# anilkeshwani/speech-integration

Measured on AMD Instinct MI355X. Metric: train_tokens_per_sec, higher is better.
Workload: dtype bf16; 1 GPU; Llama-3.2-1B +5000 DSUs (V=133258), SFT step fwd+bwd+AdamW, seq_len=2048, batch=8/GPU, grad_accum=1, 16 layers, random-init weights, MLS-shaped synthetic DSU sequences; global_batch=8, seq_len=2048, parallelism=dp1

## Files before the change

include/ssi_hip.h:

```cpp
#ifndef SSI_HIP_H
#define SSI_HIP_H

#include <stdint.h>

#ifdef __cplusplus
extern "C" {
#endif

#define SSI_ABI_VERSION 9

enum { SSI_F32 = 0, SSI_BF16 = 1 };
enum { SSI_OK = 0, SSI_ERR_ARG = 1, SSI_ERR_UNSUPPORTED = 2, SSI_ERR_WORKSPACE = 3, SSI_ERR_HIP = 1000  };
enum { SSI_GEMM_NT = 0, SSI_GEMM_NN = 1, SSI_GEMM_TN = 2 };
enum { SSI_TILES_STATIC = 0, SSI_TILES_DYNAMIC = 1 };
int ssi_set_gemm_tile_order(int mode);

enum { SSI_IMPL_AUTO = 0, SSI_IMPL_GENERIC = 1, SSI_IMPL_MFMA = 2,
       SSI_IMPL_MFMA_WG8 = 3  };

int ssi_abi_version(void);
const char* ssi_last_error(void);
int ssi_set_impl(int impl);

int ssi_embed_fwd(const int64_t* tokens, const void* table, void* out, int64_t n_tok, int64_t dim, int64_t vocab,
                  int dtype, void* stream);
int64_t ssi_embed_bwd_workspace_bytes(int64_t vocab);
int ssi_embed_bwd(const int64_t* tokens, const void* dout, void* dtable, int64_t n_tok, int64_t dim, int64_t vocab,
                  int dtype, void* workspace, int64_t workspace_bytes, void* stream);

int ssi_rmsnorm_fwd(const void* x, const void* scale, void* y, float* rstd, int64_t rows, int64_t dim, float eps,
                    int dtype, void* stream);
int64_t ssi_rmsnorm_bwd_workspace_bytes(int64_t rows, int64_t dim);
int ssi_rmsnorm_bwd(const void* dy, const void* x, const void* scale, const float* rstd, const void* dres, void* dx,
                    void* dscale, int accumulate_dscale, int64_t rows, int64_t dim, int dtype, void* workspace,
                    int64_t workspace_bytes, void* stream);

int ssi_rope_inplace(void* x, int64_t ld, int64_t rows, int64_t seq_len, int n_heads_rot, int head_dim,
                     const float* table, int64_t table_len, const int32_t* positions, int inverse, int dtype,
                     void* stream);

int ssi_gemm_rope(int64_t M, int64_t N, int64_t K, const void* A, int64_t lda, const void* B, int64_t ldb, void* C, int64_t ldc,
                  int64_t seq_len, int n_heads_rot, int head_dim, const float* rope_table, int64_t table_len,
                  const int32_t* positions, int dtype, void* stream);

int ssi_attn_fwd(const void* qkv, int64_t ld, void* out, float* lse, int64_t batch, int64_t seq, int n_heads,
                 int n_kv, int head_dim, int dtype, void* stream);
int ssi_attn_bwd(const void* qkv, int64_t ld, const void* out, const void* dout, const float* lse, void* dqkv,
                 float* delta, int64_t batch, int64_t seq, int n_heads, int n_kv, int head_dim, int dtype,
                 void* stream);

int ssi_attn_varlen_fwd(const void* qkv, int64_t ld, void* out, float* lse, const int32_t* doc_start, const int32_t* doc_end,
                        int64_t batch, int64_t seq, int n_heads, int n_kv, int head_dim, int dtype, void* stream);
int ssi_attn_varlen_bwd(const void* qkv, int64_t ld, const void* out, const void* dout, const float* lse, void* dqkv,
                        float* delta, const int32_t* doc_start, const int32_t* doc_end, int64_t batch, int64_t seq,
                        int n_heads, int n_kv, int head_dim, int dtype, void* stream);

int ssi_doc_ranges(const int64_t* input_pos, int64_t batch, int64_t seq, int64_t max_pos, int32_t* positions, int32_t* doc_start,
                   int32_t* doc_end, int32_t* n_clamped, void* stream);

// ... 81 lines not shown
```

speech-integration_amd/csrc/embed_ce.hip:

```cpp
#include "common_hip.h"

template <typename T>
__global__ __launch_bounds__(256) void embed_fwd_kernel(const int64_t* __restrict__ tokens, const T* __restrict__ table,
                                                        T* __restrict__ out, int64_t n_tok, int dim, int64_t vocab) {
    constexpr int N = Vec16<T>::N;
    const int nvec = dim / N;
    for (int64_t t = blockIdx.x; t < n_tok; t += gridDim.x) {
        const int64_t tok = tokens[t];
        const bool ok = tok >= 0 && tok < vocab;
        for (int v = threadIdx.x; v < nvec; v += 256) {
            Vec16<T> a;
            if (ok) a = load16(table + tok * dim + v * N);
            else
#pragma unroll
                for (int i = 0; i < N; ++i) a.set(i, 0.f);
            store16(out + t * dim + v * N, a);
        }
    }
}

extern "C" int ssi_embed_fwd(const int64_t* tokens, const void* table, void* out, int64_t n_tok, int64_t dim,
                             int64_t vocab, int dtype, void* stream) {
    if (n_tok == 0) return SSI_OK;
    SSI_CHECK_ARG(tokens && table && out && n_tok > 0 && dim > 0 && dim % 8 == 0 && vocab > 0);
    const unsigned grid = (unsigned)(n_tok < 65536 ? n_tok : 65536);
    SSI_DISPATCH_DTYPE(dtype, hipLaunchKernelGGL(embed_fwd_kernel<T>, dim3(grid), dim3(256), 0, (hipStream_t)stream, tokens,
                                                 (const T*)table, (T*)out, n_tok, (int)dim, vocab));
    SSI_LAUNCH_CHECK();
    return SSI_OK;
}

__global__ __launch_bounds__(256) void embed_index_kernel(const int64_t* __restrict__ tokens, int64_t n_tok, int64_t vocab,
                                                          int* __restrict__ first, int* __restrict__ count) {
    const int64_t t = (int64_t)blockIdx.x * 256 + threadIdx.x;
    if (t >= n_tok) return;
    const int64_t tok = tokens[t];
    if (tok < 0 || tok >= vocab) return;
    atomicMin(&first[tok], (int)t);
    atomicAdd(&count[tok], 1);
}

template <typename T, int MAXV>
__global__ __launch_bounds__(256) void embed_bwd_kernel(const int64_t* __restrict__ tokens, const T* __restrict__ dout,
                                                        T* __restrict__ dtable, int64_t n_tok, int dim, int64_t vocab,
                                                        const int* __restrict__ first, const int* __restrict__ count) {
    constexpr int N = Vec16<T>::N;
    const int lane = threadIdx.x & 63;
    const int64_t t0 = (int64_t)blockIdx.x * 4 + (threadIdx.x >> 6);
    if (t0 >= n_tok) return;
    const int64_t tok = tokens[t0];
    if (tok < 0 || tok >= vocab) return;
    if (first[tok] != (int)t0) return;
    const int need = count[tok];
    const int nvec = dim / N;
    float acc[MAXV][N];
#pragma unroll
    for (int k = 0; k < MAXV; ++k)
#pragma unroll
        for (int i = 0; i < N; ++i) acc[k][i] = 0.f;
    constexpr int SCAN = 8, ROWS = 8;
    __shared__ int hits_lds[4][64 * SCAN];
    int* hits = hits_lds[threadIdx.x >> 6];
    int found = 0;
    for (int64_t base0 = (t0 / 64) * 64; base0 < n_tok && found < need; base0 += 64 * SCAN) {
        int64_t tk[SCAN];
#pragma unroll
        for (int u = 0; u < SCAN; ++u) {
            const int64_t idx = base0 + 64 * u + lane;
            tk[u] = tokens[idx < n_tok ? idx : n_tok - 1];
        }
        int n = 0;
#pragma unroll
        for (int u = 0; u < SCAN; ++u) {
            const int64_t idx = base0 + 64 * u + lane;
            const bool hit = idx < n_tok && idx >= t0 && tk[u] == tok;
            const unsigned long long mask = __ballot(hit);
            if (hit) hits[n + __popcll(mask & ((1ull << lane) - 1ull))] = (int)(idx - base0);
            n += __popcll(mask);
        }
        __builtin_amdgcn_s_waitcnt(0xc07f);
        if (n == 1) {
            const T* src = dout + (base0 + hits[0]) * dim;
#pragma unroll
            for (int k = 0; k < MAXV; ++k) {
                const int v = lane + k * 64;
                const Vec16<T> r = load16(src + (v < nvec ? v : nvec - 1) * N);
#pragma unroll
                for (int i = 0; i < N; ++i) acc[k][i] += v < nvec ? r.get(i) : 0.f;
            }
        } else
        for (int h0 = 0; h0 < n; h0 += ROWS) {
            int pos[ROWS];
#pragma unroll
            for (int u = 0; u < ROWS; ++u) pos[u] = hits[h0 + u < n ? h0 + u : n - 1];
            Vec16<T> a[ROWS][MAXV];
#pragma unroll
            for (int u = 0; u < ROWS; ++u) {
                const T* src = dout + (base0 + pos[u]) * dim;
#pragma unroll
                for (int k = 0; k < MAXV; ++k) {
                    const int v = lane + k * 64;
                    a[u][k] = load16(src + (v < nvec ? v : nvec - 1) * N);
                }
            }
            __builtin_amdgcn_sched_barrier(0);
#pragma unroll
            for (int u = 0; u < ROWS; ++u) {
                const bool row_ok = h0 + u < n;
#pragma unroll
                for (int k = 0; k < MAXV; ++k) {
                    const bool ok = row_ok && lane + k * 64 < nvec;
#pragma unroll
                    for (int i = 0; i < N; ++i) acc[k][i] += ok ? a[u][k].get(i) : 0.f;
                }
            }
        }
        found += n;
    }
    T* dst = dtable + tok * dim;
#pragma unroll
    for (int k = 0; k < MAXV; ++k) {
        const int v = lane + k * 64;
        if (v < nvec) {
            Vec16<T> a = load16(dst + v * N);
#pragma unroll
            for (int i = 0; i < N; ++i) a.set(i, a.get(i) + acc[k][i]);
            store16(dst + v * N, a);
        }
    }
}

static inline int64_t embed_ws_vocab_slots(int64_t vocab) { return ssi_align_up(vocab, 64); }
extern "C" int64_t ssi_embed_bwd_workspace_bytes(int64_t vocab) { return 2 * embed_ws_vocab_slots(vocab) * (int64_t)sizeof(int); }

template <typename T>
static int launch_embed_bwd(const int64_t* tokens, const T* dout, T* dtable, int64_t n_tok, int dim, int64_t vocab,
                            const int* first, const int* count, hipStream_t st) {
    const int64_t vec_per_lane = ssi_cdiv(dim / Vec16<T>::N, 64);
    const dim3 grid((unsigned)ssi_cdiv(n_tok, 4));
    if (vec_per_lane <= 1) hipLaunchKernelGGL((embed_bwd_kernel<T, 1>), grid, dim3(256), 0, st, tokens, dout, dtable, n_tok, dim, vocab, first, count);
    else if (vec_per_lane <= 2) hipLaunchKernelGGL((embed_bwd_kernel<T, 2>), grid, dim3(256), 0, st, tokens, dout, dtable, n_tok, dim, vocab, first, count);
    else if (vec_per_lane <= 4) hipLaunchKernelGGL((embed_bwd_kernel<T, 4>), grid, dim3(256), 0, st, tokens, dout, dtable, n_tok, dim, vocab, first, count);
    else if (vec_per_lane <= 8) hipLaunchKernelGGL((embed_bwd_kernel<T, 8>), grid, dim3(256), 0, st, tokens, dout, dtable, n_tok, dim, vocab, first, count);
    else { ssi_set_error("embed_bwd: dim %d too large", dim); return SSI_ERR_UNSUPPORTED; }
    return SSI_OK;
}

extern "C" int ssi_embed_bwd(const int64_t* tokens, const void* dout, void* dtable, int64_t n_tok, int64_t dim,
                             int64_t vocab, int dtype, void* workspace, int64_t workspace_bytes, void* stream) {
    if (n_tok == 0) return SSI_OK;
    SSI_CHECK_ARG(tokens && dout && dtable && n_tok > 0 && n_tok < (1LL << 31) && dim > 0 && dim % 8 == 0 && vocab > 0);
    if (!workspace || workspace_bytes < ssi_embed_bwd_workspace_bytes(vocab)) { ssi_set_error("embed_bwd: workspace too small"); return SSI_ERR_WORKSPACE; }
    auto st = (hipStream_t)stream;
    int* first = (int*)workspace;
    int* count = first + embed_ws_vocab_slots(vocab);
    hipError_t e = hipMemsetAsync(first, 0x7f, embed_ws_vocab_slots(vocab) * sizeof(int), st);
    if (e == hipSuccess) e = hipMemsetAsync(count, 0, embed_ws_vocab_slots(vocab) * sizeof(int), st);
    if (e != hipSuccess) { ssi_set_error("embed_bwd: memset failed: %s", hipGetErrorString(e)); return SSI_ERR_HIP + (int)e; }
    hipLaunchKernelGGL(embed_index_kernel, dim3((unsigned)ssi_cdiv(n_tok, 256)), dim3(256), 0, st, tokens, n_tok, vocab, first, count);
    SSI_LAUNCH_CHECK();
    int rc = SSI_OK;
    SSI_DISPATCH_DTYPE(dtype, rc = launch_embed_bwd<T>(tokens, (const T*)dout, (T*)dtable, n_tok, (int)dim, vocab, first, count, st));
    if (rc) return rc;
    SSI_LAUNCH_CHECK();
    return SSI_OK;
}

template <typename T>
__global__ __launch_bounds__(512) void ce_fwd_kernel(T* __restrict__ logits, int64_t ld, const int64_t* __restrict__ labels,
                                                     int64_t vocab, int64_t ignore_index, float* __restrict__ row_loss,
                                                     float* __restrict__ row_lse, int write_grad, const float* __restrict__ row_weight) {
    constexpr int N = Vec16<T>::N;
    __shared__ float red[16];
    const int64_t row = blockIdx.x;
    T* lr = logits + row * ld;
    const int64_t label = labels[row];
    const bool valid = label != ignore_index && label >= 0 && label < vocab;
    const int64_t nvec = ld / N;
    if (!valid) {
        if (threadIdx.x == 0) { row_loss[row] = 0.f; if (row_lse) row_lse[row] = 0.f; }
        if (write_grad) {
            Vec16<T> z;
#pragma unroll
            for (int i = 0; i < N; ++i) z.set(i, 0.f);
            for (int64_t v = threadIdx.x; v < nvec; v += 512) store16(lr + v * N, z);
        }
        return;
    }
    float m = -INFINITY, s = 0.f;
    for (int64_t v = threadIdx.x; v < nvec; v += 512) {
        Vec16<T> a = load16(lr + v * N);
        float lm = -INFINITY;
#pragma unroll
        for (int i = 0; i < N; ++i) if (v * N + i < vocab) lm = fmaxf(lm, a.get(i));
        if (lm > m) { s *= expf(m - lm); m = lm; }
#pragma unroll
        for (int i = 0; i < N; ++i) if (v * N + i < vocab) s += expf(a.get(i) - m);
    }
// ... 196 lines not shown
```

speech-integration_amd/ssi/_lib.py:

```python

from __future__ import annotations

import ctypes
import os
from ctypes import POINTER, c_char_p, c_double, c_float, c_int, c_int32, c_int64, c_void_p

import torch

_HERE = os.path.dirname(os.path.abspath(__file__))
LIB_PATH = os.environ.get("SSI_HIP_LIB") or os.path.join(os.path.dirname(_HERE), "libssi_hip.so")

SSI_F32, SSI_BF16 = 0, 1
GEMM_NT, GEMM_NN, GEMM_TN = 0, 1, 2
IMPL_AUTO, IMPL_GENERIC, IMPL_MFMA, IMPL_MFMA_WG8 = 0, 1, 2, 3
TILES_STATIC, TILES_DYNAMIC = 0, 1
ABI_VERSION = 9
ATTN_KERNEL_DQ, ATTN_KERNEL_DKV = 0, 1
ATTN_MODE_AUTO, ATTN_MODE_OLD, ATTN_MODE_NEW, ATTN_MODE_NO_HEAD_SPLIT = 0, 1, 2, 3
ATTN_USED_DQ2, ATTN_USED_DKV2, ATTN_USED_HEAD_SPLIT, ATTN_USED_PLAN = 1, 2, 4, 8
ATTN_PLAN_HEADER, ATTN_PLAN_FORCE, ATTN_PLAN_SPLIT_ALL = 16, 1, 2

_P = c_void_p
PROTOTYPES = {
    "ssi_abi_version": (c_int, []),
    "ssi_last_error": (c_char_p, []),
    "ssi_set_impl": (c_int, [c_int]),
    "ssi_set_attn_impl": (c_int, [c_int, c_int]),
    "ssi_attn_last_dispatch": (c_int, []),
    "ssi_embed_fwd": (c_int, [_P, _P, _P, c_int64, c_int64, c_int64, c_int, _P]),
    "ssi_embed_bwd_workspace_bytes": (c_int64, [c_int64]),
    "ssi_embed_bwd": (c_int, [_P, _P, _P, c_int64, c_int64, c_int64, c_int, _P, c_int64, _P]),
    "ssi_rmsnorm_fwd": (c_int, [_P, _P, _P, _P, c_int64, c_int64, c_float, c_int, _P]),
    "ssi_rmsnorm_bwd_workspace_bytes": (c_int64, [c_int64, c_int64]),
    "ssi_rmsnorm_bwd": (c_int, [_P, _P, _P, _P, _P, _P, _P, c_int, c_int64, c_int64, c_int, _P, c_int64, _P]),
    "ssi_rope_inplace": (c_int, [_P, c_int64, c_int64, c_int64, c_int, c_int, _P, c_int64, _P, c_int, c_int, _P]),
    "ssi_gemm_rope": (c_int, [c_int64, c_int64, c_int64, _P, c_int64, _P, c_int64, _P, c_int64, c_int64, c_int, c_int, _P, c_int64, _P,
                              c_int, _P]),
    "ssi_attn_fwd": (c_int, [_P, c_int64, _P, _P, c_int64, c_int64, c_int, c_int, c_int, c_int, _P]),
    "ssi_attn_bwd": (c_int, [_P, c_int64, _P, _P, _P, _P, _P, c_int64, c_int64, c_int, c_int, c_int, c_int, _P]),
    "ssi_set_gemm_tile_order": (c_int, [c_int]),
    "ssi_attn_varlen_fwd": (c_int, [_P, c_int64, _P, _P, _P, _P, c_int64, c_int64, c_int, c_int, c_int, c_int, _P]),
    "ssi_attn_varlen_bwd": (c_int, [_P, c_int64, _P, _P, _P, _P, _P, _P, _P, c_int64, c_int64, c_int, c_int, c_int, c_int, _P]),
    "ssi_attn_varlen_bwd_rope": (c_int, [_P, c_int64, _P, _P, _P, _P, _P, _P, _P, _P, c_int64, _P, c_int64, c_int64, c_int, c_int, c_int,
                                         c_int, _P]),
    "ssi_attn_bwd_workspace_bytes": (c_int64, [c_int64, c_int64, c_int, c_int, c_int, c_int]),
    "ssi_attn_varlen_bwd_ws": (c_int, [_P, c_int64, _P, _P, _P, _P, _P, _P, _P, _P, c_int64, _P, c_int64, c_int64, c_int, c_int, c_int,
                                       c_int, _P, c_int64, _P]),
    "ssi_attn_plan_words": (c_int64, [c_int64, c_int64, c_int64]),
    "ssi_attn_plan_workspace_bytes": (c_int64, [_P]),
    "ssi_attn_plan_build": (c_int64, [_P, _P, _P, c_int64, c_int64, c_int64, c_int, c_int, c_int, _P, c_int64]),
    "ssi_attn_varlen_bwd_plan": (c_int, [_P, c_int64, _P, _P, _P, _P, _P, _P, _P, _P, c_int64, _P, c_int64, c_int64, c_int, c_int, c_int,
                                         c_int, _P, c_int64, _P, _P, _P]),
    "ssi_doc_ranges": (c_int, [_P, c_int64, c_int64, c_int64, _P, _P, _P, _P, _P]),
    "ssi_swiglu_fwd": (c_int, [_P, _P, c_int64, c_int64, c_int, _P]),
    "ssi_swiglu_bwd": (c_int, [_P, _P, _P, c_int64, c_int64, c_int, _P]),
    "ssi_gemm": (c_int, [c_int, c_int64, c_int64, c_int64, _P, c_int64, _P, c_int64, _P, c_int64, _P, c_float, _P,
                         c_int, c_int, _P]),
    "ssi_gemm_splitk_workspace_bytes": (c_int64, [c_int64, c_int64, c_int]),
    "ssi_gemm_splitk": (c_int, [c_int, c_int64, c_int64, c_int64, _P, c_int64, _P, c_int64, _P, c_int64, _P, c_float, _P,
                                c_int, c_int, c_int, _P, c_int64, _P]),
    "ssi_gemm_batched": (c_int, [c_int, c_int, c_int64, c_int64, c_int64, _P, c_int64, c_int64, _P, c_int64, c_int64, _P, c_int64, c_int64,
                                 c_float, _P, c_int, c_int, _P]),
# ... 77 lines not shown
```

speech-integration_amd/ssi/model.py:

```python

from __future__ import annotations

import os

import logging
import math
from typing import Any, Optional

import torch
from torch import Tensor, nn

from . import _lib, ops
from .constants import CROSS_ENTROPY_IGNORE_IDX, PRECISION_STR_TO_DTYPE
from .llama_configs import ConfigLlama3_2
from .ops import GEMM_NN, GEMM_NT, GEMM_TN

LOGGER = logging.getLogger(__name__)

VOCAB_ALIGN = 256


def _align(n: int, a: int) -> int:
    return (n + a - 1) // a * a

# ... 319 lines not shown
        H, KV, hd, dt, A = self.num_heads, self.num_kv_heads, self.head_dim, self.dtype, self._arena
        if pos is None and S > self._rope.shape[0]:
            raise ValueError(f"sequence length {S} exceeds the RoPE cache ({self._rope.shape[0]})")
        tok = tokens.reshape(-1).contiguous()
        L = self.num_layers
        h = A.get("h0" if save else "h0.x", (T, D), dt)
        ops.embed_fwd(tok, self._view("emb"), h, self.vocab_size)
        for l in range(L):
            sfx = f"{l}" if save else "x"
            xn1 = A.get("xn1.all", (L, T, D), dt)[l] if save else A.get("xn1.x", (T, D), dt)
            rstd1 = A.get(f"rstd1.{sfx}", (T,), torch.float32)
            ops.rmsnorm_fwd(h, self._view(f"L{l}.sa_norm"), xn1, rstd1, self.norm_eps)
            qkv = A.get(f"qkv.{sfx}", (T, self.qkv_dim), dt)
            ops.gemm_rope(xn1, self._view(f"L{l}.wqkv"), qkv, S, H + KV, hd, self._rope, positions=pos)
            att = A.get("att.all", (L, T, H * hd), dt)[l] if save else A.get("att.x", (T, H * hd), dt)
            lse = A.get(f"lse.{sfx}", (B * H * S,), torch.float32)
            ops.attn_fwd(qkv, att, lse, B, S, H, KV, hd, ds, de)
            hmid = A.get(f"hmid.{sfx}", (T, D), dt)
            self._gemm(GEMM_NT, att, self._view(f"L{l}.wo"), hmid, residual=h)
            xn2 = A.get(f"xn2.{sfx}", (T, D), dt)
            rstd2 = A.get(f"rstd2.{sfx}", (T,), torch.float32)
            ops.rmsnorm_fwd(hmid, self._view(f"L{l}.mlp_norm"), xn2, rstd2, self.norm_eps)
            gu = A.get(f"gu.{sfx}", (T, 2 * I), dt)
            act = A.get(f"act.{sfx}", (T, I), dt)
            ops.gemm_swiglu_fwd(xn2, self._view(f"L{l}.w13"), gu, act)
            hn_name = f"h{l + 1}" if save else f"hx{l & 1}"
            hnext = A.get(hn_name, (T, D), dt)
            self._gemm(GEMM_NT, act, self._view(f"L{l}.w2"), hnext, residual=hmid)
            h = hnext
        hn = A.get("hn" if save else "hn.x", (T, D), dt)
        rstdf = A.get("rstdf" if save else "rstdf.x", (T,), torch.float32)
        ops.rmsnorm_fwd(h, self.norm.scale, hn, rstdf, self.norm_eps)
        if save:
            self._fwd_generation += 1
            self._saved = {"tok": tok, "B": B, "S": S, "gen": self._fwd_generation, "pos": pos, "ds": ds, "de": de, "plan": plan}
        return hn

    def _backward_hidden(self, d_hn: Tensor, gen: int) -> None:
        sv = self._saved
        if sv is None or sv["gen"] != gen:
            raise RuntimeError("HipLlamaDecoder: backward called for a forward whose activations were overwritten; "
                               "run backward before the next training forward")
        B, S, tok = sv["B"], sv["S"], sv["tok"]
        pos, ds, de, plan = sv["pos"], sv["ds"], sv["de"], sv.get("plan")
        T, D, I = B * S, self.embed_dim, self.intermediate_dim
        H, KV, hd, dt, A = self.num_heads, self.num_kv_heads, self.head_dim, self.dtype, self._arena
        L = self.num_layers
        G = self._flat_grad
        self._finish_pending_exchange()
        acc = self._window_accumulates()
        gv = lambda name: self._view(name, None, G)
        ws = A.get("ws.rms", (max(ops.rmsnorm_bwd_workspace_bytes(T, D), 16),), torch.uint8)

        def wgrad(dy: Tensor, x: Tensor, name: str) -> None:
            g = gv(name)
            splits = ops.splitk_choice(g.shape[0], g.shape[1], T) if (dt == torch.bfloat16 and T % 64 == 0) else 1
            if splits > 1:
                wsk = A.get("ws.splitk", (splits * g.shape[0] * g.shape[1],), torch.float32)
                ops.gemm_splitk(GEMM_TN, dy, x, g, splits, wsk, accumulate=acc)
            else:
                ops.gemm(GEMM_TN, dy, x, g, accumulate=acc)

        sync = self.grad_sync if (self.grad_sync is not None and self.sync_this_backward) else None
        listener, self.bucket_listener = (self.bucket_listener if self.sync_this_backward else None), None

        def announce(name: str) -> None:
            if sync:
                sync.bucket_ready(*self._bucket_by_name[name])
            if listener is not None:
                listener(*self._bucket_by_name[name])

        Gp = self.wgrad_group
        if sync and Gp != self._bucket_group:
            raise RuntimeError("wgrad_group was changed after construction: the data-parallel buckets were laid out for the old grouping")
        defer = (Gp > 1 and dt == torch.bfloat16 and self._mfma_shapes() and T % 128 == 0 and T >= 256
                 and ops.splitk_choice(D, H * hd, T) > 1 and ops.splitk_choice(self.qkv_dim, D, T) > 1)
        xn1_all, att_all = A.get("xn1.all", (L, T, D), dt), A.get("att.all", (L, T, H * hd), dt)
        if defer:
            dhmid_all, dqkv_all = A.get("dh.b.all", (Gp, T, D), dt), A.get("dqkv.all", (Gp, T, self.qkv_dim), dt)
            lstride = (self._slices["L1.wqkv"][0] - self._slices["L0.wqkv"][0]) if L > 1 else 0

        def flush_attention_wgrads(l_lo: int) -> None:
            n = min(Gp, L - l_lo)
            g_o = torch.as_strided(G, (n, D, H * hd), (lstride, H * hd, 1), self._slices[f"L{l_lo}.wo"][0])
            g_qkv = torch.as_strided(G, (n, self.qkv_dim, D), (lstride, D, 1), self._slices[f"L{l_lo}.wqkv"][0])
            ops.gemm_batched(GEMM_TN, dhmid_all[:n], att_all[l_lo:l_lo + n], g_o, accumulate=acc)
            ops.gemm_batched(GEMM_TN, dqkv_all[:n], xn1_all[l_lo:l_lo + n], g_qkv, accumulate=acc)

        def dgrad(dy: Tensor, name: str, dx: Tensor) -> None:
            self._gemm(GEMM_NN, dy, self._view(name), dx)

        ws_bytes = ops.attn_bwd_workspace_bytes(B, S, H, KV, hd, dt) if T > 0 else 0
        if plan is not None:
            ws_bytes = max(ws_bytes, plan.workspace_bytes)
        attn_ws = A.get("ws.attn", (ws_bytes,), torch.uint8) if ws_bytes else None
        dh = A.get("dh.a", (T, D), dt)
        ops.rmsnorm_bwd(d_hn, A.get(f"h{L}", (T, D), dt), self.norm.scale, A.get("rstdf", (T,), torch.float32), None, dh,
                        gv("norm"), ws, accumulate=acc)
        announce("norm")
        for l in reversed(range(L)):
            xn1, xn2 = xn1_all[l], A.get(f"xn2.{l}", (T, D), dt)
            qkv, att = A.get(f"qkv.{l}", (T, self.qkv_dim), dt), att_all[l]
            hmid, gu, act = A.get(f"hmid.{l}", (T, D), dt), A.get(f"gu.{l}", (T, 2 * I), dt), A.get(f"act.{l}", (T, I), dt)
            h_in = A.get(f"h{l}", (T, D), dt)
            wgrad(dh, act, f"L{l}.w2")
            dgu = A.get("dgu", (T, 2 * I), dt)
            ops.gemm_swiglu_bwd(GEMM_NN, dh, self._view(f"L{l}.w2"), gu, dgu, A.get("dact", (T, I), dt))
            dxn = A.get("dxn", (T, D), dt)
            dgrad(dgu, f"L{l}.w13", dxn)
            wgrad(dgu, xn2, f"L{l}.w13")
            dhmid = dhmid_all[l % Gp] if defer else A.get("dh.b", (T, D), dt)
            ops.rmsnorm_bwd(dxn, hmid, self._view(f"L{l}.mlp_norm"), A.get(f"rstd2.{l}", (T,), torch.float32), dh, dhmid,
                            gv(f"L{l}.mlp_norm"), ws, accumulate=acc)
            datt = A.get("datt", (T, H * hd), dt)
            dgrad(dhmid, f"L{l}.wo", datt)
            if not defer:
                wgrad(dhmid, att, f"L{l}.wo")
            dqkv = dqkv_all[l % Gp] if defer else A.get("dqkv", (T, self.qkv_dim), dt)
            delta = A.get("delta", (B * H * S,), torch.float32)
            ops.attn_bwd(qkv, att, datt, A.get(f"lse.{l}", (B * H * S,), torch.float32), dqkv, delta, B, S, H, KV, hd, ds, de,
                         rope_table=self._rope, positions=pos, workspace=attn_ws, plan=plan)
            dgrad(dqkv, f"L{l}.wqkv", dxn)
            if not defer:
                wgrad(dqkv, xn1, f"L{l}.wqkv")
            ops.rmsnorm_bwd(dxn, h_in, self._view(f"L{l}.sa_norm"), A.get(f"rstd1.{l}", (T,), torch.float32), dhmid, dh,
                            gv(f"L{l}.sa_norm"), ws, accumulate=acc)
            announce(f"L{l}.mlp")
            if defer and l % Gp == 0:
                flush_attention_wgrads(l)
            if l % self._bucket_group == 0:
                announce(f"attn.{l}")
        ws_e = A.get("ws.emb", (max(_lib.load().ssi_embed_bwd_workspace_bytes(self.vocab_size), 16),), torch.uint8)
        if not acc and not self._emb_grad_written:
            gv("emb").zero_()
        ops.embed_bwd(tok, dh, gv("emb"), self.vocab_size, ws_e)
        self._grads_dirty, self._grads_stale, self._emb_grad_written = True, False, False
        announce("emb")
        self._saved = None
        self.attach_grads()

    def _head_logits(self, hn: Tensor, arena_name: Optional[str] = None) -> Tensor:
        T = hn.shape[0]
        if arena_name is None:
            logits = torch.empty((T, self.vocab_pad), dtype=self.dtype, device=self.device)
        else:
            logits = self._arena.get(arena_name, (T, self.vocab_pad), self.dtype)
        ops.gemm(GEMM_NT, hn, self._view("emb"), logits)
        return logits

    def _head_backward(self, dlogits: Tensor, hn: Tensor, alpha_dev: Optional[Tensor]) -> Tensor:
        T, D = hn.shape
        self._finish_pending_exchange()
        acc = self._window_accumulates()
        d_hn = self._arena.get("d_hn", (T, D), self.dtype)
        ops.gemm(GEMM_NN, dlogits, self._view("emb"), d_hn, alpha_dev=alpha_dev)
        g_emb = self._view("emb", None, self._flat_grad)
        rows_main = self._head_wgrad_main_rows(T)
        if rows_main:
            Vp = self.vocab_pad
            ops.gemm(GEMM_TN, dlogits[:, :rows_main], hn, g_emb[:rows_main], alpha_dev=alpha_dev, accumulate=acc)
            tail, splits = Vp - rows_main, self._head_wgrad_tail_splits
            wsk = self._arena.get("ws.splitk.head", (splits * tail * D,), torch.float32)
            ops.gemm_splitk(GEMM_TN, dlogits[:, rows_main:], hn, g_emb[rows_main:], splits, wsk, alpha_dev=alpha_dev, accumulate=acc)
        else:
            ops.gemm(GEMM_TN, dlogits, hn, g_emb, alpha_dev=alpha_dev, accumulate=acc)
        self._emb_grad_written = True
        return d_hn

# ... 194 lines not shown
```

speech-integration_amd/ssi/ops.py:

```python

from __future__ import annotations

import torch
from typing import Optional
from torch import Tensor

from . import _lib
from ._lib import GEMM_NN, GEMM_NT, GEMM_TN, check, dtype_code, ptr, stream_ptr

__all__ = ["lmhead_ce_fwd", "lmhead_ce_bwd", "doc_ranges", "embed_fwd", "embed_bwd", "rmsnorm_fwd", "rmsnorm_bwd", "rope_", "attn_fwd", "attn_bwd", "attn_bwd_workspace_bytes", "swiglu_fwd",
           "swiglu_bwd", "gemm", "gemm_splitk", "splitk_choice", "gemm_swiglu_fwd", "gemm_swiglu_bwd", "transpose", "ce_fwd", "ce_reduce", "count_tokens", "scale_", "sumsq", "adamw_step", "set_impl", "set_attn_impl", "attn_last_dispatch",
           "GEMM_NT", "GEMM_NN", "GEMM_TN"]


def set_impl(impl: int) -> int:
    return _lib.load().ssi_set_impl(impl)


def set_attn_impl(which: int, mode: int) -> int:
    return _lib.load().ssi_set_attn_impl(which, mode)


def attn_last_dispatch() -> int:
    return _lib.load().ssi_attn_last_dispatch()


def _byte_ws(nbytes: int, like: Tensor) -> Tensor:
    return torch.empty(max(int(nbytes), 16), dtype=torch.uint8, device=like.device)


def embed_fwd(tokens: Tensor, table: Tensor, out: Tensor, vocab: int) -> None:
    n, dim = tokens.numel(), table.shape[1]
    assert tokens.dtype == torch.int64 and tokens.is_contiguous() and out.is_contiguous() and table.stride(1) == 1
    assert table.stride(0) == dim and out.shape[-1] == dim and out.numel() == n * dim and out.dtype == table.dtype
    check(_lib.load().ssi_embed_fwd(ptr(tokens), ptr(table), ptr(out), n, dim, vocab, dtype_code(table.dtype),
                                    stream_ptr()), "ssi_embed_fwd")


def embed_bwd(tokens: Tensor, dout: Tensor, dtable: Tensor, vocab: int, workspace: Tensor | None = None) -> None:
    lib = _lib.load()
    n, dim = tokens.numel(), dtable.shape[1]
    assert tokens.dtype == torch.int64 and tokens.is_contiguous() and dout.is_contiguous() and dtable.stride(0) == dim
    need = lib.ssi_embed_bwd_workspace_bytes(vocab)
    if workspace is None or workspace.numel() * workspace.element_size() < need:
        workspace = _byte_ws(need, dout)
    check(lib.ssi_embed_bwd(ptr(tokens), ptr(dout), ptr(dtable), n, dim, vocab, dtype_code(dtable.dtype), ptr(workspace),
                            workspace.numel() * workspace.element_size(), stream_ptr()), "ssi_embed_bwd")


def rmsnorm_fwd(x: Tensor, scale: Tensor, y: Tensor, rstd: Tensor | None, eps: float) -> None:
    dim = x.shape[-1]
    rows = x.numel() // dim
    assert x.is_contiguous() and y.is_contiguous() and scale.is_contiguous() and scale.numel() == dim
    assert rstd is None or (rstd.dtype == torch.float32 and rstd.numel() >= rows)
    check(_lib.load().ssi_rmsnorm_fwd(ptr(x), ptr(scale), ptr(y), ptr(rstd), rows, dim, eps, dtype_code(x.dtype),
                                      stream_ptr()), "ssi_rmsnorm_fwd")


def rmsnorm_bwd_workspace_bytes(rows: int, dim: int) -> int:
    return _lib.load().ssi_rmsnorm_bwd_workspace_bytes(rows, dim)


def rmsnorm_bwd(dy: Tensor, x: Tensor, scale: Tensor, rstd: Tensor, dres: Tensor | None, dx: Tensor, dscale: Tensor,
                workspace: Tensor | None = None, accumulate: bool = True) -> None:
    lib = _lib.load()
    dim = x.shape[-1]
    rows = x.numel() // dim
    assert dy.is_contiguous() and x.is_contiguous() and dx.is_contiguous() and dscale.is_contiguous()
    assert dres is None or dres.is_contiguous()
    need = lib.ssi_rmsnorm_bwd_workspace_bytes(rows, dim)
    if workspace is None or workspace.numel() * workspace.element_size() < need:
        workspace = _byte_ws(need, dy)
    check(lib.ssi_rmsnorm_bwd(ptr(dy), ptr(x), ptr(scale), ptr(rstd), ptr(dres), ptr(dx), ptr(dscale), int(accumulate), rows, dim,
                              dtype_code(x.dtype), ptr(workspace), workspace.numel() * workspace.element_size(),
                              stream_ptr()), "ssi_rmsnorm_bwd")


def rope_(x: Tensor, seq_len: int, n_heads_rot: int, head_dim: int, table: Tensor, inverse: bool = False,
          positions: Tensor | None = None) -> None:
    assert x.dim() == 2 and x.stride(1) == 1 and table.dtype == torch.float32 and table.is_contiguous()
# ... 288 lines not shown
```

Measured before the change: 159,000 tokens/s.

## Replace atomic embedding-backward index with sorted segment plan built during forward

Embedding backward no longer memsets two vocab-sized arrays and has each first-occurrence wave scan the token stream for duplicates. A plan (a stable rank sort of token ids plus per-token segments) is now built in the forward pass, on a side stream when one is available. Backward then runs a scatter kernel with one block per unique token, summing its rows without atomics. The embedding gradient is also issued right after layer 0's rmsnorm backward. The cost moves to an O(n^2/64) rank-counting sort and a single-block segment kernel in forward, plus cross-stream synchronization.

```diff
diff --git a/include/ssi_hip.h b/include/ssi_hip.h
--- a/include/ssi_hip.h
+++ b/include/ssi_hip.h
@@ -7,7 +7,7 @@
 extern "C" {
 #endif
 
-#define SSI_ABI_VERSION 9
+#define SSI_ABI_VERSION 10
 
 enum { SSI_F32 = 0, SSI_BF16 = 1 };
 enum { SSI_OK = 0, SSI_ERR_ARG = 1, SSI_ERR_UNSUPPORTED = 2, SSI_ERR_WORKSPACE = 3, SSI_ERR_HIP = 1000  };
@@ -24,7 +24,10 @@
 
 int ssi_embed_fwd(const int64_t* tokens, const void* table, void* out, int64_t n_tok, int64_t dim, int64_t vocab,
                   int dtype, void* stream);
-int64_t ssi_embed_bwd_workspace_bytes(int64_t vocab);
+int64_t ssi_embed_plan_bytes(int64_t n_tok);
+int ssi_embed_plan_build(const int64_t* tokens, int64_t n_tok, int64_t vocab, void* plan, int64_t plan_bytes, void* stream);
+int ssi_embed_bwd_planned(const void* plan, const void* dout, void* dtable, int64_t n_tok, int64_t dim, int dtype, void* stream);
+int64_t ssi_embed_bwd_workspace_bytes(int64_t n_tok);
 int ssi_embed_bwd(const int64_t* tokens, const void* dout, void* dtable, int64_t n_tok, int64_t dim, int64_t vocab,
                   int dtype, void* workspace, int64_t workspace_bytes, void* stream);
 
diff --git a/speech-integration_amd/csrc/embed_ce.hip b/speech-integration_amd/csrc/embed_ce.hip
--- a/speech-integration_amd/csrc/embed_ce.hip
+++ b/speech-integration_amd/csrc/embed_ce.hip
@@ -30,140 +30,191 @@
     return SSI_OK;
 }
 
-__global__ __launch_bounds__(256) void embed_index_kernel(const int64_t* __restrict__ tokens, int64_t n_tok, int64_t vocab,
-                                                          int* __restrict__ first, int* __restrict__ count) {
-    const int64_t t = (int64_t)blockIdx.x * 256 + threadIdx.x;
-    if (t >= n_tok) return;
-    const int64_t tok = tokens[t];
-    if (tok < 0 || tok >= vocab) return;
-    atomicMin(&first[tok], (int)t);
-    atomicAdd(&count[tok], 1);
-}
-
-template <typename T, int MAXV>
-__global__ __launch_bounds__(256) void embed_bwd_kernel(const int64_t* __restrict__ tokens, const T* __restrict__ dout,
-                                                        T* __restrict__ dtable, int64_t n_tok, int dim, int64_t vocab,
-                                                        const int* __restrict__ first, const int* __restrict__ count) {
+static inline int64_t embed_plan_pitch(int64_t n_tok) { return ssi_align_up(n_tok + 1, 64); }
+extern "C" int64_t ssi_embed_plan_bytes(int64_t n_tok) { return n_tok < 0 ? 0 : (4 + 5 * embed_plan_pitch(n_tok)) * (int64_t)sizeof(int); }
+
+constexpr int PLAN_ID_NONE = 0x7fffffff;
+
+__global__ __launch_bounds__(256) void embed_plan_ids_kernel(const int64_t* __restrict__ tokens, int n_tok, int64_t vocab,
+                                                             int* __restrict__ ids, int pitch) {
+    const int t = blockIdx.x * 256 + threadIdx.x;
+    if (t >= pitch) return;
+    int id = PLAN_ID_NONE;
+    if (t < n_tok) {
+        const int64_t tok = tokens[t];
+        if (tok >= 0 && tok < vocab) id = (int)tok;
+    }
+    ids[t] = id;
+}
+
+__global__ __launch_bounds__(512) void embed_plan_place_kernel(const int* __restrict__ ids, int n_tok, int* __restrict__ order,
+                                                               int* __restrict__ sorted_id) {
+    __shared__ int part[8][64];
+    const int lane = threadIdx.x & 63, wave = __builtin_amdgcn_readfirstlane(threadIdx.x >> 6);
+    const int own = blockIdx.x, t = own * 64 + lane;
+    const int my = t < n_tok ? ids[t] : PLAN_ID_NONE;
+    const int groups = (n_tok + 63) >> 6;
+    int place = 0;
+    for (int g = wave; g < own; g += 8) {
+        const int* q = ids + 64 * g;
+#pragma unroll
+        for (int k = 0; k < 64; ++k) place += q[k] <= my;
+    }
+    for (int g = own + 1 + wave; g < groups; g += 8) {
+        const int* q = ids + 64 * g;
+#pragma unroll
+        for (int k = 0; k < 64; ++k) place += q[k] < my;
+    }
+    if (wave == 0) {
+        const int* q = ids + 64 * own;
+#pragma unroll
+        for (int k = 0; k < 64; ++k) place += q[k] < my || (q[k] == my && k < lane);
+    }
+    part[wave][lane] = place;
+    __syncthreads();
+    if (wave == 0 && my != PLAN_ID_NONE) {
+        int s = 0;
+#pragma unroll
+        for (int w = 0; w < 8; ++w) s += part[w][lane];
+        order[s] = t;
+        sorted_id[s] = my;
+    }
+}
+
+__global__ __launch_bounds__(256) void embed_plan_segments_kernel(const int* __restrict__ ids, int n_tok, const int* __restrict__ sorted_id,
+                                                                  int* __restrict__ header, int* __restrict__ seg_start,
+                                                                  int* __restrict__ seg_token) {
+    __shared__ int wsum[4];
+    const int lane = threadIdx.x & 63, wave = threadIdx.x >> 6;
+    int n = 0;
+    for (int t = threadIdx.x; t < n_tok; t += 256) n += ids[t] != PLAN_ID_NONE;
+#pragma unroll
+    for (int o = 32; o > 0; o >>= 1) n += __shfl_xor(n, o, 64);
+    if (lane == 0) wsum[wave] = n;
+    __syncthreads();
+    const int n_valid = wsum[0] + wsum[1] + wsum[2] + wsum[3];
+    int base = 0;
+    for (int i0 = 0; i0 < n_valid; i0 += 1024) {
+        const int i = i0 + 4 * threadIdx.x;
+        int id[4];
+        bool head[4];
+        int last = i > 0 && i <= n_valid ? sorted_id[i - 1] : -1, heads = 0;
+#pragma unroll
+        for (int k = 0; k < 4; ++k) {
+            id[k] = i + k < n_valid ? sorted_id[i + k] : 0;
+            head[k] = i + k < n_valid && (i + k == 0 || id[k] != last);
+            heads += head[k];
+            last = id[k];
+        }
+        int upto = heads;
+#pragma unroll
+        for (int o = 1; o < 64; o <<= 1) {
+            const int below = __shfl_up(upto, o, 64);
+            if (lane >= o) upto += below;
+        }
+        __syncthreads();
+        if (lane == 63) wsum[wave] = upto;
+        __syncthreads();
+        int u = base + upto - heads;
+#pragma unroll
+        for (int w = 0; w < 4; ++w) u += w < wave ? wsum[w] : 0;
+#pragma unroll
+        for (int k = 0; k < 4; ++k)
+            if (head[k]) {
+                seg_start[u] = i + k;
+                seg_token[u] = id[k];
+                ++u;
+            }
+        base += wsum[0] + wsum[1] + wsum[2] + wsum[3];
+    }
+    if (threadIdx.x == 0) {
+        header[0] = base; header[1] = n_valid; header[2] = 0; header[3] = 0;
+        seg_start[base] = n_valid;
+    }
+}
+
+extern "C" int ssi_embed_plan_build(const int64_t* tokens, int64_t n_tok, int64_t vocab, void* plan, int64_t plan_bytes, void* stream) {
+    SSI_CHECK_ARG(n_tok >= 0 && n_tok < (1LL << 31) - 64 && vocab > 0 && vocab < PLAN_ID_NONE && plan && (tokens || n_tok == 0) &&
+                  ((uintptr_t)plan % 16) == 0);
+    if (plan_bytes < ssi_embed_plan_bytes(n_tok)) { ssi_set_error("embed_plan: plan buffer too small"); return SSI_ERR_WORKSPACE; }
+    auto st = (hipStream_t)stream;
+    const int64_t P = embed_plan_pitch(n_tok);
+    int* header = (int*)plan;
+    int *order = header + 4, *seg_start = order + P, *seg_token = seg_start + P, *sorted_id = seg_token + P, *ids = sorted_id + P;
+    hipLaunchKernelGGL(embed_plan_ids_kernel, dim3((unsigned)ssi_cdiv(P, 256)), dim3(256), 0, st, tokens, (int)n_tok, vocab, ids, (int)P);
+    SSI_LAUNCH_CHECK();
+    if (n_tok > 0) {
+        hipLaunchKernelGGL(embed_plan_place_kernel, dim3((unsigned)ssi_cdiv(n_tok, 64)), dim3(512), 0, st, ids, (int)n_tok, order, sorted_id);
+        SSI_LAUNCH_CHECK();
+    }
+    hipLaunchKernelGGL(embed_plan_segments_kernel, dim3(1), dim3(256), 0, st, ids, (int)n_tok, sorted_id, header, seg_start, seg_token);
+    SSI_LAUNCH_CHECK();
+    return SSI_OK;
+}
+
+template <typename T, int R, bool CLAMP>
+__device__ __forceinline__ void embed_add_rows(float (&acc)[Vec16<T>::N], const T* __restrict__ col, const int* __restrict__ order, int r,
+                                               int hi, int dim) {
+    Vec16<T> a[R];
+#pragma unroll
+    for (int k = 0; k < R; ++k) a[k] = load16(col + (int64_t)order[CLAMP && r + k >= hi ? hi - 1 : r + k] * dim);
+    __builtin_amdgcn_sched_barrier(0);
+#pragma unroll
+    for (int k = 0; k < R; ++k) {
+        const bool ok = !CLAMP || r + k < hi;
+#pragma unroll
+        for (int i = 0; i < Vec16<T>::N; ++i) acc[i] += ok ? a[k].get(i) : 0.f;
+    }
+}
+
+template <typename T>
+__global__ __launch_bounds__(256) void embed_scatter_kernel(const int* __restrict__ plan, int64_t pitch, const T* __restrict__ dout,
+                                                            T* __restrict__ dtable, int dim) {
     constexpr int N = Vec16<T>::N;
-    const int lane = threadIdx.x & 63;
-    const int64_t t0 = (int64_t)blockIdx.x * 4 + (threadIdx.x >> 6);
-    if (t0 >= n_tok) return;
-    const int64_t tok = tokens[t0];
-    if (tok < 0 || tok >= vocab) return;
-    if (first[tok] != (int)t0) return;
-    const int need = count[tok];
+    const int u = blockIdx.x;
+    if (u >= plan[0]) return;
+    const int* order = plan + 4;
+    const int* seg_start = order + pitch;
+    const int* seg_token = seg_start + pitch;
+    const int lo = seg_start[u], hi = seg_start[u + 1];
+    const int64_t tok = seg_token[u];
     const int nvec = dim / N;
-    float acc[MAXV][N];
-#pragma unroll
-    for (int k = 0; k < MAXV; ++k)
-#pragma unroll
-        for (int i = 0; i < N; ++i) acc[k][i] = 0.f;
-    constexpr int SCAN = 8, ROWS = 8;
-    __shared__ int hits_lds[4][64 * SCAN];
-    int* hits = hits_lds[threadIdx.x >> 6];
-    int found = 0;
-    for (int64_t base0 = (t0 / 64) * 64; base0 < n_tok && found < need; base0 += 64 * SCAN) {
-        int64_t tk[SCAN];
-#pragma unroll
-        for (int u = 0; u < SCAN; ++u) {
-            const int64_t idx = base0 + 64 * u + lane;
-            tk[u] = tokens[idx < n_tok ? idx : n_tok - 1];
-        }
-        int n = 0;
-#pragma unroll
-        for (int u = 0; u < SCAN; ++u) {
-            const int64_t idx = base0 + 64 * u + lane;
-            const bool hit = idx < n_tok && idx >= t0 && tk[u] == tok;
-            const unsigned long long mask = __ballot(hit);
-            if (hit) hits[n + __popcll(mask & ((1ull << lane) - 1ull))] = (int)(idx - base0);
-            n += __popcll(mask);
-        }
-        __builtin_amdgcn_s_waitcnt(0xc07f);
-        if (n == 1) {
-            const T* src = dout + (base0 + hits[0]) * dim;
-#pragma unroll
-            for (int k = 0; k < MAXV; ++k) {
-                const int v = lane + k * 64;
-                const Vec16<T> r = load16(src + (v < nvec ? v : nvec - 1) * N);
-#pragma unroll
-                for (int i = 0; i < N; ++i) acc[k][i] += v < nvec ? r.get(i) : 0.f;
-            }
-        } else
-        for (int h0 = 0; h0 < n; h0 += ROWS) {
-            int pos[ROWS];
-#pragma unroll
-            for (int u = 0; u < ROWS; ++u) pos[u] = hits[h0 + u < n ? h0 + u : n - 1];
-            Vec16<T> a[ROWS][MAXV];
-#pragma unroll
-            for (int u = 0; u < ROWS; ++u) {
-                const T* src = dout + (base0 + pos[u]) * dim;
-#pragma unroll
-                for (int k = 0; k < MAXV; ++k) {
-                    const int v = lane + k * 64;
-                    a[u][k] = load16(src + (v < nvec ? v : nvec - 1) * N);
-                }
-            }
-            __builtin_amdgcn_sched_barrier(0);
-#pragma unroll
-            for (int u = 0; u < ROWS; ++u) {
-                const bool row_ok = h0 + u < n;
-#pragma unroll
-                for (int k = 0; k < MAXV; ++k) {
-                    const bool ok = row_ok && lane + k * 64 < nvec;
-#pragma unroll
-                    for (int i = 0; i < N; ++i) acc[k][i] += ok ? a[u][k].get(i) : 0.f;
-                }
-            }
-        }
-        found += n;
-    }
-    T* dst = dtable + tok * dim;
-#pragma unroll
-    for (int k = 0; k < MAXV; ++k) {
-        const int v = lane + k * 64;
-        if (v < nvec) {
-            Vec16<T> a = load16(dst + v * N);
-#pragma unroll
-            for (int i = 0; i < N; ++i) a.set(i, a.get(i) + acc[k][i]);
-            store16(dst + v * N, a);
-        }
-    }
-}
-
-static inline int64_t embed_ws_vocab_slots(int64_t vocab) { return ssi_align_up(vocab, 64); }
-extern "C" int64_t ssi_embed_bwd_workspace_bytes(int64_t vocab) { return 2 * embed_ws_vocab_slots(vocab) * (int64_t)sizeof(int); }
-
-template <typename T>
-static int launch_embed_bwd(const int64_t* tokens, const T* dout, T* dtable, int64_t n_tok, int dim, int64_t vocab,
-                            const int* first, const int* count, hipStream_t st) {
-    const int64_t vec_per_lane = ssi_cdiv(dim / Vec16<T>::N, 64);
-    const dim3 grid((unsigned)ssi_cdiv(n_tok, 4));
-    if (vec_per_lane <= 1) hipLaunchKernelGGL((embed_bwd_kernel<T, 1>), grid, dim3(256), 0, st, tokens, dout, dtable, n_tok, dim, vocab, first, count);
-    else if (vec_per_lane <= 2) hipLaunchKernelGGL((embed_bwd_kernel<T, 2>), grid, dim3(256), 0, st, tokens, dout, dtable, n_tok, dim, vocab, first, count);
-    else if (vec_per_lane <= 4) hipLaunchKernelGGL((embed_bwd_kernel<T, 4>), grid, dim3(256), 0, st, tokens, dout, dtable, n_tok, dim, vocab, first, count);
-    else if (vec_per_lane <= 8) hipLaunchKernelGGL((embed_bwd_kernel<T, 8>), grid, dim3(256), 0, st, tokens, dout, dtable, n_tok, dim, vocab, first, count);
-    else { ssi_set_error("embed_bwd: dim %d too large", dim); return SSI_ERR_UNSUPPORTED; }
+    for (int v = threadIdx.x; v < nvec; v += 256) {
+        float acc[N];
+#pragma unroll
+        for (int i = 0; i < N; ++i) acc[i] = 0.f;
+        const T* col = dout + (int64_t)v * N;
+        int r = lo;
+        for (; r + 32 <= hi; r += 32) embed_add_rows<T, 32, false>(acc, col, order, r, hi, dim);
+        for (; r + 8 <= hi; r += 8) embed_add_rows<T, 8, false>(acc, col, order, r, hi, dim);
+        for (; r < hi; r += 4) embed_add_rows<T, 4, true>(acc, col, order, r, hi, dim);
+        T* dst = dtable + tok * dim + (int64_t)v * N;
+        Vec16<T> g = load16(dst);
+#pragma unroll
+        for (int i = 0; i < N; ++i) g.set(i, g.get(i) + acc[i]);
+        store16(dst, g);
+    }
+}
+
+extern "C" int ssi_embed_bwd_planned(const void* plan, const void* dout, void* dtable, int64_t n_tok, int64_t dim, int dtype,
+                                     void* stream) {
+    if (n_tok == 0) return SSI_OK;
+    SSI_CHECK_ARG(plan && dout && dtable && n_tok > 0 && n_tok < (1LL << 31) && dim > 0 && dim % 8 == 0 && ((uintptr_t)plan % 16) == 0);
+    SSI_DISPATCH_DTYPE(dtype, hipLaunchKernelGGL(embed_scatter_kernel<T>, dim3((unsigned)n_tok), dim3(256), 0, (hipStream_t)stream,
+                                                 (const int*)plan, embed_plan_pitch(n_tok), (const T*)dout, (T*)dtable, (int)dim));
+    SSI_LAUNCH_CHECK();
     return SSI_OK;
 }
+
+extern "C" int64_t ssi_embed_bwd_workspace_bytes(int64_t n_tok) { return ssi_embed_plan_bytes(n_tok); }
 
 extern "C" int ssi_embed_bwd(const int64_t* tokens, const void* dout, void* dtable, int64_t n_tok, int64_t dim,
                              int64_t vocab, int dtype, void* workspace, int64_t workspace_bytes, void* stream) {
     if (n_tok == 0) return SSI_OK;
     SSI_CHECK_ARG(tokens && dout && dtable && n_tok > 0 && n_tok < (1LL << 31) && dim > 0 && dim % 8 == 0 && vocab > 0);
-    if (!workspace || workspace_bytes < ssi_embed_bwd_workspace_bytes(vocab)) { ssi_set_error("embed_bwd: workspace too small"); return SSI_ERR_WORKSPACE; }
-    auto st = (hipStream_t)stream;
-    int* first = (int*)workspace;
-    int* count = first + embed_ws_vocab_slots(vocab);
-    hipError_t e = hipMemsetAsync(first, 0x7f, embed_ws_vocab_slots(vocab) * sizeof(int), st);
-    if (e == hipSuccess) e = hipMemsetAsync(count, 0, embed_ws_vocab_slots(vocab) * sizeof(int), st);
-    if (e != hipSuccess) { ssi_set_error("embed_bwd: memset failed: %s", hipGetErrorString(e)); return SSI_ERR_HIP + (int)e; }
-    hipLaunchKernelGGL(embed_index_kernel, dim3((unsigned)ssi_cdiv(n_tok, 256)), dim3(256), 0, st, tokens, n_tok, vocab, first, count);
-    SSI_LAUNCH_CHECK();
-    int rc = SSI_OK;
-    SSI_DISPATCH_DTYPE(dtype, rc = launch_embed_bwd<T>(tokens, (const T*)dout, (T*)dtable, n_tok, (int)dim, vocab, first, count, st));
-    if (rc) return rc;
-    SSI_LAUNCH_CHECK();
-    return SSI_OK;
+    if (!workspace || workspace_bytes < ssi_embed_bwd_workspace_bytes(n_tok)) { ssi_set_error("embed_bwd: workspace too small"); return SSI_ERR_WORKSPACE; }
+    if (int rc = ssi_embed_plan_build(tokens, n_tok, vocab, workspace, workspace_bytes, stream)) return rc;
+    return ssi_embed_bwd_planned(workspace, dout, dtable, n_tok, dim, dtype, stream);
 }
 
 template <typename T>
diff --git a/speech-integration_amd/ssi/_lib.py b/speech-integration_amd/ssi/_lib.py
--- a/speech-integration_amd/ssi/_lib.py
+++ b/speech-integration_amd/ssi/_lib.py
@@ -14,7 +14,7 @@
 GEMM_NT, GEMM_NN, GEMM_TN = 0, 1, 2
 IMPL_AUTO, IMPL_GENERIC, IMPL_MFMA, IMPL_MFMA_WG8 = 0, 1, 2, 3
 TILES_STATIC, TILES_DYNAMIC = 0, 1
-ABI_VERSION = 9
+ABI_VERSION = 10
 ATTN_KERNEL_DQ, ATTN_KERNEL_DKV = 0, 1
 ATTN_MODE_AUTO, ATTN_MODE_OLD, ATTN_MODE_NEW, ATTN_MODE_NO_HEAD_SPLIT = 0, 1, 2, 3
 ATTN_USED_DQ2, ATTN_USED_DKV2, ATTN_USED_HEAD_SPLIT, ATTN_USED_PLAN = 1, 2, 4, 8
@@ -28,6 +28,9 @@
     "ssi_set_attn_impl": (c_int, [c_int, c_int]),
     "ssi_attn_last_dispatch": (c_int, []),
     "ssi_embed_fwd": (c_int, [_P, _P, _P, c_int64, c_int64, c_int64, c_int, _P]),
+    "ssi_embed_plan_bytes": (c_int64, [c_int64]),
+    "ssi_embed_plan_build": (c_int, [_P, c_int64, c_int64, _P, c_int64, _P]),
+    "ssi_embed_bwd_planned": (c_int, [_P, _P, _P, c_int64, c_int64, c_int, _P]),
     "ssi_embed_bwd_workspace_bytes": (c_int64, [c_int64]),
     "ssi_embed_bwd": (c_int, [_P, _P, _P, c_int64, c_int64, c_int64, c_int, _P, c_int64, _P]),
     "ssi_rmsnorm_fwd": (c_int, [_P, _P, _P, _P, c_int64, c_int64, c_float, c_int, _P]),
diff --git a/speech-integration_amd/ssi/model.py b/speech-integration_amd/ssi/model.py
--- a/speech-integration_amd/ssi/model.py
+++ b/speech-integration_amd/ssi/model.py
@@ -375,9 +375,26 @@
         rstdf = A.get("rstdf" if save else "rstdf.x", (T,), torch.float32)
         ops.rmsnorm_fwd(h, self.norm.scale, hn, rstdf, self.norm_eps)
         if save:
+            eplan = self._build_embed_plan(tok)
             self._fwd_generation += 1
-            self._saved = {"tok": tok, "B": B, "S": S, "gen": self._fwd_generation, "pos": pos, "ds": ds, "de": de, "plan": plan}
+            self._saved = {"tok": tok, "B": B, "S": S, "gen": self._fwd_generation, "pos": pos, "ds": ds, "de": de, "plan": plan, "eplan": eplan}
         return hn
+
+    def _build_embed_plan(self, tok: Tensor) -> tuple[Tensor, Optional[torch.cuda.Event]]:
+        plan = self._arena.get("emb.plan", (ops.embed_plan_words(tok.numel()),), torch.int32)
+        opt = self._hip_optimizer() if getattr(self, "_hip_optimizer", None) is not None else None
+        side = getattr(opt, "_side", None) if self.grad_sync is None else None
+        if side is None:
+            ops.embed_plan(tok, self.vocab_size, plan)
+            return plan, None
+        side.wait_stream(torch.cuda.current_stream(self.device))
+        with torch.cuda.stream(side):
+            ops.embed_plan(tok, self.vocab_size, plan)
+            ready = torch.cuda.Event()
+            ready.record(side)
+        for t in (tok, plan):
+            t.record_stream(side)
+        return plan, ready
 
     def _backward_hidden(self, d_hn: Tensor, gen: int) -> None:
         sv = self._saved
@@ -438,6 +455,15 @@
             ws_bytes = max(ws_bytes, plan.workspace_bytes)
         attn_ws = A.get("ws.attn", (ws_bytes,), torch.uint8) if ws_bytes else None
         dh = A.get("dh.a", (T, D), dt)
+
+        def embedding_grad() -> None:
+            if not acc and not self._emb_grad_written:
+                gv("emb").zero_()
+            eplan, eplan_ready = sv["eplan"]
+            if eplan_ready is not None:
+                torch.cuda.current_stream(self.device).wait_event(eplan_ready)
+            ops.embed_bwd_planned(eplan, dh, gv("emb"))
+
         ops.rmsnorm_bwd(d_hn, A.get(f"h{L}", (T, D), dt), self.norm.scale, A.get("rstdf", (T,), torch.float32), None, dh,
                         gv("norm"), ws, accumulate=acc)
         announce("norm")
@@ -468,15 +494,15 @@
                 wgrad(dqkv, xn1, f"L{l}.wqkv")
             ops.rmsnorm_bwd(dxn, h_in, self._view(f"L{l}.sa_norm"), A.get(f"rstd1.{l}", (T,), torch.float32), dhmid, dh,
                             gv(f"L{l}.sa_norm"), ws, accumulate=acc)
+            if l == 0:
+                embedding_grad()
             announce(f"L{l}.mlp")
             if defer and l % Gp == 0:
                 flush_attention_wgrads(l)
             if l % self._bucket_group == 0:
                 announce(f"attn.{l}")
-        ws_e = A.get("ws.emb", (max(_lib.load().ssi_embed_bwd_workspace_bytes(self.vocab_size), 16),), torch.uint8)
-        if not acc and not self._emb_grad_written:
-            gv("emb").zero_()
-        ops.embed_bwd(tok, dh, gv("emb"), self.vocab_size, ws_e)
+        if L == 0:
+            embedding_grad()
         self._grads_dirty, self._grads_stale, self._emb_grad_written = True, False, False
         announce("emb")
         self._saved = None
diff --git a/speech-integration_amd/ssi/ops.py b/speech-integration_amd/ssi/ops.py
--- a/speech-integration_amd/ssi/ops.py
+++ b/speech-integration_amd/ssi/ops.py
@@ -8,7 +8,7 @@
 from . import _lib
 from ._lib import GEMM_NN, GEMM_NT, GEMM_TN, check, dtype_code, ptr, stream_ptr
 
-__all__ = ["lmhead_ce_fwd", "lmhead_ce_bwd", "doc_ranges", "embed_fwd", "embed_bwd", "rmsnorm_fwd", "rmsnorm_bwd", "rope_", "attn_fwd", "attn_bwd", "attn_bwd_workspace_bytes", "swiglu_fwd",
+__all__ = ["lmhead_ce_fwd", "lmhead_ce_bwd", "doc_ranges", "embed_fwd", "embed_bwd", "embed_plan_words", "embed_plan", "embed_plan_views", "embed_bwd_planned", "rmsnorm_fwd", "rmsnorm_bwd", "rope_", "attn_fwd", "attn_bwd", "attn_bwd_workspace_bytes", "swiglu_fwd",
            "swiglu_bwd", "gemm", "gemm_splitk", "splitk_choice", "gemm_swiglu_fwd", "gemm_swiglu_bwd", "transpose", "ce_fwd", "ce_reduce", "count_tokens", "scale_", "sumsq", "adamw_step", "set_impl", "set_attn_impl", "attn_last_dispatch",
            "GEMM_NT", "GEMM_NN", "GEMM_TN"]
 
@@ -41,11 +41,34 @@
     lib = _lib.load()
     n, dim = tokens.numel(), dtable.shape[1]
     assert tokens.dtype == torch.int64 and tokens.is_contiguous() and dout.is_contiguous() and dtable.stride(0) == dim
-    need = lib.ssi_embed_bwd_workspace_bytes(vocab)
+    need = lib.ssi_embed_bwd_workspace_bytes(n)
     if workspace is None or workspace.numel() * workspace.element_size() < need:
         workspace = _byte_ws(need, dout)
     check(lib.ssi_embed_bwd(ptr(tokens), ptr(dout), ptr(dtable), n, dim, vocab, dtype_code(dtable.dtype), ptr(workspace),
                             workspace.numel() * workspace.element_size(), stream_ptr()), "ssi_embed_bwd")
+
+
+def embed_plan_words(n_tok: int) -> int:
+    return _lib.load().ssi_embed_plan_bytes(n_tok) // 4
+
+
+def embed_plan(tokens: Tensor, vocab: int, plan: Tensor) -> None:
+    assert tokens.dtype == torch.int64 and tokens.is_contiguous() and plan.dtype == torch.int32 and plan.is_contiguous()
+    check(_lib.load().ssi_embed_plan_build(ptr(tokens) if tokens.numel() else None, tokens.numel(), vocab, ptr(plan), plan.numel() * 4,
+                                           stream_ptr()), "ssi_embed_plan_build")
+
+
+def embed_plan_views(plan: Tensor, n_tok: int) -> dict[str, Tensor]:
+    P = (n_tok + 1 + 63) // 64 * 64
+    return {"header": plan[:4], "order": plan[4:4 + P], "seg_start": plan[4 + P:4 + 2 * P], "seg_token": plan[4 + 2 * P:4 + 3 * P]}
+
+
+def embed_bwd_planned(plan: Tensor, dout: Tensor, dtable: Tensor) -> None:
+    n, dim = dout.shape[0], dtable.shape[1]
+    assert plan.dtype == torch.int32 and plan.numel() >= embed_plan_words(n) and dout.is_contiguous() and dout.shape[1] == dim
+    assert dtable.stride(0) == dim and dout.dtype == dtable.dtype
+    check(_lib.load().ssi_embed_bwd_planned(ptr(plan), ptr(dout), ptr(dtable), n, dim, dtype_code(dtable.dtype), stream_ptr()),
+          "ssi_embed_bwd_planned")
 
 
 def rmsnorm_fwd(x: Tensor, scale: Tensor, y: Tensor, rstd: Tensor | None, eps: float) -> None:
```

New measurement: 159,300 tokens/s, median of 6. About the same (+0.2%).
